# Gepetto/mpc-interface

Measured on AMD Instinct MI355X. Metric: QP assemblies/sec (P,q,G,h), biped N=16 batched, higher is better.
Workload: dtype f64; 1 GPU; C2 biped LIPM N=16 no=36 nc=76, per-instance (A,B)/given/aim, K1 on chip; batch_per_gpu=4096, global_batch=4096, streams=2

## Files before the change

### include/mpcasm.h

```cpp
#ifndef MPCASM_H
#define MPCASM_H

#include <stddef.h>
#include <stdint.h>

#ifdef __cplusplus
extern "C" {
#endif

typedef enum mpcasm_status {
  MPCASM_OK = 0,
  MPCASM_ERR_ARG = -1,
  MPCASM_ERR_PLAN = -2,
  MPCASM_ERR_HIP = -3,
  MPCASM_ERR_NODEVICE = -4,
  MPCASM_ERR_LIMIT = -5
} mpcasm_status;

typedef struct mpcasm_plan mpcasm_plan;


int mpcasm_abi_version(void);
int mpcasm_device_count(void);
int mpcasm_last_hip(void);
const char* mpcasm_status_string(int status);
enum { MPCASM_OPT_PATH = 1, MPCASM_OPT_PHASE_MASK = 2, MPCASM_OPT_RESIDENT_PER_CU = 3, MPCASM_OPT_JIT = 4,
       MPCASM_OPT_P_DIRECT = 5, MPCASM_OPT_RESIDENT_GRID = 6, MPCASM_OPT_JIT_FETCH_RUNS = 7 };
int mpcasm_set_option(int option, int value);
int mpcasm_plan_set_option(mpcasm_plan* plan, int option, int value);
int mpcasm_resident_lds_bytes(const int32_t* h_itab, size_t n_itab, const double* h_dtab, size_t n_dtab,
                              int64_t out[2]);
int mpcasm_jit_check(const int32_t* h_itab, size_t n_itab, const double* h_dtab, size_t n_dtab,
                     char* log, size_t log_capacity);
int mpcasm_fetch_segments(const int32_t* h_itab, size_t n_itab, const double* h_dtab, size_t n_dtab,
                          int limit, int32_t* out, size_t capacity, int64_t* n_words);

int mpcasm_plan_prepare(const mpcasm_plan* plan, int batch);
int mpcasm_jit_stats(int64_t out[3]);

int mpcasm_fill_su(const double* d_A, const double* d_B, double* d_S, double* d_U,
                   int batch, int N, int n, int m, int ltv, void* stream);

// ... 41 lines not shown
                         double* d_out, int batch, void* stream);

int mpcasm_preview_goal_distance(const mpcasm_plan* plan, const double* const* h_src,
                                 const int64_t* h_src_stride, const double* d_given,
                                 const double* d_optim, const double* d_params, const int32_t* d_terms,
                                 int nterms, int ngoals, double* d_out, void* d_work, int batch,
                                 void* stream);

enum { MPCASM_PREVIEW_NONE = 0 , MPCASM_PREVIEW_DIRECT = 1,
       MPCASM_PREVIEW_STAGED = 2 ,
       MPCASM_PREVIEW_BLOCKED = 3  };
int mpcasm_preview_route(const int32_t* h_itab, size_t n_itab, const double* h_dtab, size_t n_dtab,
                         const int64_t* h_src_stride, int nterms, int ngoals, int32_t out[8]);

int mpcasm_sweep_route(const int32_t* h_itab, size_t n_itab, const double* h_dtab, size_t n_dtab, int32_t out[8]);

enum { MPCASM_TILED_SCAN = 1, MPCASM_TILED_TOEPLITZ = 2, MPCASM_TILED_SHARED = 3, MPCASM_TILED_GENERAL = 4 };
enum { MPCASM_TILED_TABLES_NONE = 0, MPCASM_TILED_TABLES_SMALL = 1 ,
       MPCASM_TILED_TABLES_SYSTEM = 2  };
enum { MPCASM_WANT_COST = 1, MPCASM_WANT_CONSTRAINTS = 2 };
int mpcasm_tiled_route(const int32_t* h_itab, size_t n_itab, const double* h_dtab, size_t n_dtab,
                       const int64_t* h_src_stride, int batch, int want, int path, int32_t out[16]);

int mpcasm_gather(const double* d_src, int64_t src_stride, const int32_t* d_index, int nnz,
                  double* d_dst, int batch, void* stream);

enum { MPCASM_BOX_RECENTER = 0, MPCASM_BOX_TRANSLATE, MPCASM_BOX_ROTATE, MPCASM_BOX_SCALE,
       MPCASM_BOX_MARGIN };
int mpcasm_box_transform(double* d_params, int64_t n_params, int batch, const int32_t* d_facets,
                         int nfacets, int op, const double* d_arg, int64_t arg_stride,
// ... 66 lines not shown
```

### mpc-interface_amd/csrc/capi.hip

```cpp
#include <hip/hip_runtime.h>
#include <stdint.h>
#include <stdlib.h>
#include <string.h>

#include <algorithm>
#include <cmath>
#include <mutex>
#include <new>
#include <string>
#include <vector>

#include "jit.h"
#include "kernels.h"

using namespace mpcasm;

namespace mpcasm {
int g_p_direct = 0;
extern int g_path;
extern int g_phase_mask;
extern int g_resident_per_cu, g_resident_grid;
}

struct mpcasm_plan {
// ... 1065 lines not shown
  if (option == MPCASM_OPT_RESIDENT_PER_CU) {
    if (value < 0 || value > 16) return MPCASM_ERR_ARG;
    g_resident_per_cu = value;
    return MPCASM_OK;
  }
  if (option == MPCASM_OPT_JIT_FETCH_RUNS) {
    if (value < 0 || value > FS_MAX) return MPCASM_ERR_ARG;
    g_jit_fetch_runs = value;
    return MPCASM_OK;
  }
  if (option == MPCASM_OPT_RESIDENT_GRID) {
    if (value < 0 || value > (1 << 20)) return MPCASM_ERR_ARG;
    g_resident_grid = value;
    return MPCASM_OK;
  }
  return MPCASM_ERR_ARG;
}

int mpcasm_plan_set_option(mpcasm_plan* plan, int option, int value) {
  if (!plan) return MPCASM_ERR_ARG;
  if (option == MPCASM_OPT_PATH && value >= -1 && value <= 4) plan->opt_path = value;
  else if (option == MPCASM_OPT_JIT && value >= -1 && value <= 2) plan->opt_jit = value;
  else if (option == MPCASM_OPT_RESIDENT_PER_CU && value >= -1 && value <= 16) plan->opt_per_cu = value;
  else if (option == MPCASM_OPT_RESIDENT_GRID && value >= -1 && value <= (1 << 20)) plan->opt_grid = value;
  else return MPCASM_ERR_ARG;
  return MPCASM_OK;
}

const char* mpcasm_status_string(int status) {
  switch (status) {
// ... 349 lines not shown
  PlanDev d;
  memset(&d, 0, sizeof d);
  plan_dev_from_tables(h_itab, &d);
  if (!sweep_eligible(d)) return MPCASM_ERR_ARG;
  SweepChoice c;
  const int choice = sweep_choose(d, h_itab, &c);
  if (choice != MPCASM_OK) return choice;
  out[0] = c.cpt;
  out[1] = c.specialised;
  out[2] = c.pair;
  out[3] = c.per_line;
  out[4] = c.reg_lines;
  out[5] = sweep_lines_ahead(c.cpt);
  out[6] = (int32_t)c.lds;
  out[7] = c.lds > 64 * 1024;
  return MPCASM_OK;
}

int mpcasm_tiled_route(const int32_t* h_itab, size_t n_itab, const double* h_dtab, size_t n_dtab,
                       const int64_t* h_src_stride, int batch, int want, int path, int32_t out[16]) {
  if (!h_itab || (n_dtab && !h_dtab) || !out || batch < 1 || path < -1 || path > 4 || want < 1 || want > 3)
    return MPCASM_ERR_ARG;
  memset(out, 0, 16 * sizeof(int32_t));
  const int rc = validate_plan(h_itab, h_dtab, n_itab, n_dtab);
  if (rc != MPCASM_OK) return rc;
  PlanDev d;
  memset(&d, 0, sizeof d);
  plan_dev_from_tables(h_itab, &d);
  if (d.nsrc && !h_src_stride) return MPCASM_ERR_ARG;
  SrcTable src;
// ... 386 lines not shown
```

### mpc-interface_amd/csrc/kernels.h

```cpp
#pragma once
#include <hip/hip_runtime.h>
#include <stddef.h>
#include <stdint.h>

#include <vector>

#include "../../include/mpcasm.h"
#include "plan_dev.h"
#include "plan_tables.h"

namespace mpcasm {

constexpr int CU_LDS_BYTES = 160 * 1024;
hipError_t allow_whole_lds(const void* fn);

int launch_fill_su(const double* A, const double* B, double* S, double* U, int batch, int N, int n,
                   int m, int ltv, hipStream_t stream, hipError_t* err);

size_t assemble_workspace_bytes(const PlanDev& p, int batch);
int launch_assemble_staged(const PlanDev& p, const SrcTable& src, const double* params,
                           const double* given, double* P, double* q, double* G, double* h,
                           void* work, int batch, hipStream_t stream, hipError_t* err);
bool tiled_eligible(const PlanDev& p);
size_t tiled_workspace_bytes(const PlanDev& p, int batch);
// ... 4 lines not shown
int launch_lti_tables(const PlanDev& p, const SrcTable& src, double* work, int batch,
                      const int32_t* h_itab, SrcTable* eff, hipStream_t stream);
int toeplitz_zero_pad(int N);
struct TiledChoice {
  int form, fused, kp, cb, rows_in_lds, whole_lines, tables, tg, sym;
  int dlen;
  size_t lds;
};
int tiled_choose(const PlanDev& p, const SrcTable& src, const int32_t* h_itab, int path, int batch,
                 bool want_cost, bool want_constraints, bool have_given, bool have_work, TiledChoice* out);
int lti_effective_sources(const PlanDev& p, const SrcTable& src, double* work, const int32_t* h_itab,
                          SrcTable* eff);
bool sweep_eligible(const PlanDev& p);
struct SweepChoice {
  int cpt, specialised, pair, per_line, reg_lines;
  size_t lds;
};
int sweep_choose(const PlanDev& p, const int32_t* h_itab, SweepChoice* out);
int sweep_lines_ahead(int cpt);
int launch_assemble_sweep(const PlanDev& p, const SrcTable& src, const double* params,
                          const double* given, double* P, double* q, double* G, double* h, int batch,
                          hipStream_t stream, hipError_t* err, const int32_t* h_itab);
int launch_preview_direct(const PlanDev& p, const SrcTable& eff, const double* given,
                          const double* optim, double* out, int batch, int num_cus,
                          hipStream_t stream, hipError_t* err, const int32_t* h_itab = nullptr);
int launch_preview_goals(const PlanDev& p, const SrcTable& eff, const double* given, const double* optim,
                         const double* params, long long nparams, const int32_t* terms, int nterms,
                         int ngoals, double* out, int batch, int num_cus, hipStream_t stream,
                         hipError_t* err, const int32_t* h_itab);
int preview_route(const PlanDev& p, const SrcTable& eff, const int32_t* h_itab, int nterms, int ngoals,
                  int32_t out[8]);
int launch_next_given(const PlanDev& p, const SrcTable& eff, const int32_t* map, long long map_words,
// ... 65 lines not shown
```

### mpc-interface_amd/csrc/sweep.hip

```cpp
#include <hip/hip_runtime.h>
#include <stdint.h>

#include <algorithm>

#include "device_common.h"
#include "kernels.h"

namespace mpcasm {

namespace {

constexpr int SW_BLOCK = 256;
constexpr int SW_WAVES = SW_BLOCK / 64;

__device__ __forceinline__ double ldsd(const double* base, int i) { return base[i]; }

struct SweepLds {
  int ab, xbar, gv, lam, par, cvec, lw, ints, total;
  int i_term, i_gptr, i_axis, i_lword, nints;
};
constexpr int LIMW = SW_LIM_WORDS + SW_AXMAX * SW_LAX_WORDS;
constexpr int SW_TERMS_REG = 8;
constexpr int SW_LINES_REG = 8;
constexpr int sweep_lr(int cpt) { return cpt == 1 ? SW_LINES_REG : (cpt == 2 ? 4 : 2); }
__host__ __device__ inline int sweep_abw(int n, int m) { return (n * n + n * m + 1) & ~1; }
__host__ __device__ inline SweepLds sweep_lds(const PlanDev& p, int per_line) {
  const int n = p.sw_n, m = p.sw_m, N = p.sw_horizon, naxes = p.sw_naxes;
  SweepLds x;
  x.ab = 0;
  x.gv = x.ab + N * sweep_abw(n, m);
  x.lw = x.gv + naxes * m * N * SW_NMAX;
  x.xbar = x.lw + (per_line ? p.sw_ngent : p.sw_nlim) * naxes * SW_NMAX;
  x.lam = x.xbar;
  x.par = x.lam + naxes * N * n;
  x.cvec = x.par + p.nparams + 1;
  x.cvec += x.cvec & 1;
  x.ints = x.cvec + p.sw_ncvec * SW_NMAX;
  x.ints += x.ints & 1;
  x.i_term = 0;
  x.i_gptr = x.i_term + p.sw_nterm * SW_TERM_WORDS;
  x.i_axis = x.i_gptr + N + 2;
  x.i_lword = x.i_axis + naxes * SW_AXIS_WORDS;
  x.nints = x.i_lword + p.sw_ngent + SW_LINES_REG;
  x.total = x.ints + (x.nints + 1) / 2;
  x.total += x.total & 1;
  return x;
}

__device__ __forceinline__ double lane_value(double v, int src) { return __shfl(v, src, 64); }

template <int CPT, int NS, int MS, int AS, bool PAIR = false>
__global__ __launch_bounds__(SW_BLOCK) void ltv_sweep_kernel(
    PlanDev p, const double* __restrict__ sysA, long long strideA, const double* __restrict__ sysB,
    long long strideB, const double* __restrict__ params, const double* __restrict__ given,
    double* __restrict__ P, double* __restrict__ q, double* __restrict__ G, double* __restrict__ h,
    int batch, int per_line, int reg_lines) {
  extern __shared__ __attribute__((aligned(16))) double sw[];
  const int tid = threadIdx.x, lane = tid & 63;
  const int wave = __builtin_amdgcn_readfirstlane(tid >> 6);
  const long inst = blockIdx.x;
  if (inst >= batch) return;
  const int n = NS ? NS : p.sw_n, m = MS ? MS : p.sw_m, naxes = AS ? AS : p.sw_naxes;
  const int N = p.sw_horizon, no = p.no, nc = p.nc;
  const int nn = n * n, nm = n * m, abw = sweep_abw(n, m);
  const SweepLds L = sweep_lds(p, per_line);
  double* AB = sw + L.ab;
  double* xbar = sw + L.xbar;
  double* gv = sw + L.gv;
  double* lamT = sw + L.lam;
  double* par = sw + L.par;
  double* cvec = sw + L.cvec;
  double* lw = sw + L.lw;
  int* itb = reinterpret_cast<int*>(sw + L.ints);
// ... 14 lines not shown
    for (int e = tid; e <= p.nparams; e += SW_BLOCK) par[e] = e < p.nparams ? pb[e] : 0.0;
    for (int e = tid; e < p.sw_ncvec * SW_NMAX; e += SW_BLOCK) cvec[e] = (p.dtab + p.sw_doff_cvec)[e];
    auto copy = [&](int dst, int src_off, int count) {
      for (int e = tid; e < count; e += SW_BLOCK) itb[dst + e] = (p.itab + src_off)[e];
    };
    copy(L.i_term, p.off_sw_term, p.sw_nterm * SW_TERM_WORDS);
    copy(L.i_gptr, p.off_sw_gptr, N + 1);
    if (tid == 0) itb[L.i_gptr + N + 1] = nlines;
    copy(L.i_axis, p.off_sw_axis, naxes * SW_AXIS_WORDS);
  }
  int ca[CPT], cj[CPT], cl[CPT];
  double dPc[CPT], dqc[CPT];
  const int32_t* colw = p.itab + p.off_sw_col;
#pragma unroll
  for (int t = 0; t < CPT; ++t) {
    const int c = PAIR ? tid * CPT + t : tid + t * SW_BLOCK;
    ca[t] = -1;
    cj[t] = cl[t] = 0;
    dPc[t] = dqc[t] = 0.0;
    if (c < no) {
      const int w = colw[c];
      ca[t] = w & 255;
      cj[t] = (w >> 8) & 255;
      cl[t] = w >> 16;
      diagonal_of_column(p, pb, c, dPc[t], dqc[t]);
    }
  }
  __syncthreads();

  const int ra = lane >> 4, ri = (lane >> 2) & 3, rj = lane & 3;
  const bool rlive = ra < naxes && ri < n && rj < n;
// ... 158 lines not shown
        if (l + 1 < N) {
          const double* An = AB + (l + 1) * abw;
          double acl[SW_NMAX];
#pragma unroll
          for (int s_ = 0; s_ < SW_NMAX; ++s_) acl[s_] = (xl && s_ < n) ? An[s_ * n + ri] : 0.0;
          acc = fma(acl[0], lane_value(lam, base), acc);
          acc = fma(acl[1], lane_value(lam, base + 4), acc);
          acc = fma(acl[2], lane_value(lam, base + 8), acc);
          acc = fma(acl[3], lane_value(lam, base + 12), acc);
        }
        lam = xl ? acc : 0.0;
        if (xl) lamT[(ra * N + l) * n + ri] = lam;
      }
    }
  }
  if (G != nullptr && wave >= 2) {
    const int wt = tid - 128, WT = SW_BLOCK - 128;
    for (int e = wt; e < nlines + SW_LINES_REG; e += WT) {
      const int2 ge = gent[e < nlines ? e : nlines - 1];
      const int* rec = lims + ge.x * LIMW;
      lword[e] = (rec[SL_OUT0] + ge.y) | (ge.x << 20);
      if (per_line && e < nlines) {
        for (int a = 0; a < naxes; ++a)
          for (int s_ = 0; s_ < SW_NMAX; ++s_) lw[(e * naxes + a) * SW_NMAX + s_] = 0.0;
        for (int ax = 0; ax < rec[SL_NAXES]; ++ax) {
          const int* xr = rec + SW_LIM_WORDS + ax * SW_LAX_WORDS;
          const double ar = par[xr[SX_ARROW] + ge.y * xr[SX_ARROW_STEP]];
          const double* cv = cvec + xr[SX_CVEC];
          for (int s_ = 0; s_ < n; ++s_) lw[(e * naxes + xr[SX_AXIS]) * SW_NMAX + s_] += ar * cv[s_];
        }
      }
// ... 1 lines not shown
    if (!per_line)
      for (int li = wt; li < p.sw_nlim; li += WT) {
        const int* rec = lims + li * LIMW;
        for (int a = 0; a < naxes; ++a)
          for (int s_ = 0; s_ < SW_NMAX; ++s_) lw[(li * naxes + a) * SW_NMAX + s_] = 0.0;
        for (int ax = 0; ax < rec[SL_NAXES]; ++ax) {
          const int* xr = rec + SW_LIM_WORDS + ax * SW_LAX_WORDS;
          const double ar = par[xr[SX_ARROW]];
          const double* cv = cvec + xr[SX_CVEC];
          for (int s_ = 0; s_ < n; ++s_) lw[(li * naxes + xr[SX_AXIS]) * SW_NMAX + s_] += ar * cv[s_];
        }
      }
  }
  __syncthreads();

  if (P != nullptr)
#pragma unroll
    for (int t = 0; t < CPT; ++t) {
      const int c = PAIR ? tid * CPT + t : tid + t * SW_BLOCK;
      if (c < no) {
        const double* Bl = AB + cl[t] * abw + nn;
        const double* lm = lamT + (ca[t] * N + cl[t]) * n;
        double acc = dqc[t];
        for (int s_ = 0; s_ < n; ++s_) acc = fma(Bl[s_ * m + cj[t]], lm[s_], acc);
        q[(size_t)inst * no + c] = acc;
      }
    }

  double* Pb = P + (size_t)inst * no * no;
  double* Gb = G + (size_t)inst * nc * no;
  if (P != nullptr && naxes > 1) {
    const bool wide = (N & 1) == 0 && (no & 1) == 0;
    for (int a = 0; a < naxes; ++a)
      for (int j = 0; j < m; ++j)
        for (int a2 = 0; a2 < naxes; ++a2) {
          if (a2 == a) continue;
          for (int j2 = 0; j2 < m; ++j2) {
            const int col0 = axis[a2 * SW_AXIS_WORDS + 1 + j2];
            double* blk = Pb + (size_t)axis[a * SW_AXIS_WORDS + 1 + j] * no + col0;
            if (wide && (col0 & 1) == 0)
              for (int e = tid * 2; e < N * N; e += SW_BLOCK * 2) {
                const int r = e / N, c = e - r * N;
                *reinterpret_cast<double2*>(blk + (size_t)r * no + c) = double2{0.0, 0.0};
              }
            else
              for (int e = tid; e < N * N; e += SW_BLOCK) {
                const int r = e / N, c = e - r * N;
                blk[(size_t)r * no + c] = 0.0;
              }
          }
        }
  }

  if ((CPT == 1 && tid >= no) || (PAIR && tid * CPT >= no)) return;
  double u[CPT][SW_NMAX];
  double* prow[CPT][SW_MMAX];
  int goff[CPT];
#pragma unroll
  for (int t = 0; t < CPT; ++t) {
    const int c = PAIR ? tid * CPT + t : tid + t * SW_BLOCK;
    const int cat = ca[t] < 0 ? 0 : ca[t];
    goff[t] = cat * m * SW_NMAX;
#pragma unroll
    for (int i = 0; i < SW_NMAX; ++i) u[t][i] = 0.0;
#pragma unroll
    for (int j = 0; j < SW_MMAX; ++j)
      prow[t][j] = Pb + (size_t)(j < m ? axis[cat * SW_AXIS_WORDS + 1 + j] : 0) * no + (c < no ? c : 0);
  }
  constexpr int RLMAX = 4;
  double wreg[RLMAX][CPT][SW_NMAX];
  double* gp[RLMAX];
#pragma unroll
  for (int x = 0; x < RLMAX; ++x) {
    const int word = (G != nullptr && x < reg_lines) ? __builtin_amdgcn_readfirstlane(lword[x]) : 0;
    gp[x] = Gb + (size_t)(word & 0xFFFFF) * no;
#pragma unroll
    for (int t = 0; t < CPT; ++t) {
      const double* wp = lw + (size_t)(word >> 20) * naxes * SW_NMAX + (goff[t] / m);
#pragma unroll
      for (int s_ = 0; s_ < SW_NMAX; ++s_) wreg[x][t][s_] = (x < reg_lines && s_ < n) ? wp[s_] : 0.0;
    }
  }
  constexpr int LR = sweep_lr(CPT);
  int wcur[LR];
#pragma unroll
  for (int x = 0; x < LR; ++x) wcur[x] = G != nullptr ? __builtin_amdgcn_readfirstlane(lword[x]) : 0;
  int e1 = G != nullptr ? __builtin_amdgcn_readfirstlane(gptr[1]) : 0, e0 = 0;
  for (int l = 0; l < N; ++l) {
    const double* Al = AB + l * abw;
    const double* Bl = Al + nn;
    const int e2 = gptr[l + 2];
    double am[SW_NMAX][SW_NMAX];
#pragma unroll
    for (int i = 0; i < SW_NMAX; ++i)
#pragma unroll
      for (int s_ = 0; s_ < SW_NMAX; ++s_) am[i][s_] = (i < n && s_ < n) ? Al[i * n + s_] : 0.0;
#pragma unroll
    for (int t = 0; t < CPT; ++t) {
      double bnow[SW_NMAX], y[SW_NMAX];
#pragma unroll
      for (int i = 0; i < SW_NMAX; ++i) {
        bnow[i] = i < n ? Bl[i * m + cj[t]] : 0.0;
        asm volatile("" : "+v"(bnow[i]));
// ... 13 lines not shown
    }
    if (P != nullptr) {
      double pv[CPT][SW_MMAX];
#pragma unroll
      for (int t = 0; t < CPT; ++t) {
        const double* gl = gv + (size_t)l * naxes * m * SW_NMAX + goff[t];
#pragma unroll
        for (int j = 0; j < SW_MMAX; ++j) {
          double v = (cl[t] == l && cj[t] == j) ? dPc[t] : 0.0;
#pragma unroll
          for (int s_ = 0; s_ < SW_NMAX; ++s_)
            if (s_ < n && j < m) v = fma(gl[j * SW_NMAX + s_], u[t][s_], v);
          pv[t][j] = v;
        }
      }
#pragma unroll
      for (int j = 0; j < SW_MMAX; ++j) {
        if (j >= m) break;
        if constexpr (PAIR) {
          const bool m0 = cl[0] <= l, m1 = cl[1] <= l;
          if (m0 && m1 && prow[1][j] == prow[0][j] + 1) {
            *reinterpret_cast<double2*>(prow[0][j]) = double2{pv[0][j], pv[1][j]};
          } else {
            if (m0) *prow[0][j] = pv[0][j];
            if (m1) *prow[1][j] = pv[1][j];
          }
        } else {
#pragma unroll
          for (int t = 0; t < CPT; ++t) {
            const int c = tid + t * SW_BLOCK;
            if ((CPT == 1 || c < no) && cl[t] <= l) *prow[t][j] = pv[t][j];
          }
        }
#pragma unroll
        for (int t = 0; t < CPT; ++t) prow[t][j] += no;
      }
    }
    if (G != nullptr && reg_lines > 0) {
#pragma unroll
      for (int x = 0; x < RLMAX; ++x) {
        if (x >= reg_lines) break;
        double vv[CPT];
#pragma unroll
        for (int t = 0; t < CPT; ++t) {
          vv[t] = 0.0;
#pragma unroll
          for (int s_ = 0; s_ < SW_NMAX; ++s_)
            if (s_ < n) vv[t] = fma(wreg[x][t][s_], u[t][s_], vv[t]);
        }
        if constexpr (PAIR) {
          store_result(reinterpret_cast<double2*>(gp[x] + tid * 2), double2{vv[0], vv[1]});
        } else {
#pragma unroll
          for (int t = 0; t < CPT; ++t) {
            const int c = tid + t * SW_BLOCK;
            if (CPT == 1 || c < no) store_result(gp[x] + c, vv[t]);
          }
        }
        gp[x] += no;
      }
      for (int e = e0 + reg_lines; e < e1; ++e) {
        const int word = lword[e];
        double* grow = Gb + (size_t)(word & 0xFFFFF) * no;
#pragma unroll
        for (int t = 0; t < CPT; ++t) {
          const int c = PAIR ? tid * CPT + t : tid + t * SW_BLOCK;
          const double* wp = lw + (size_t)(word >> 20) * naxes * SW_NMAX + (goff[t] / m);
          double v = 0.0;
          for (int s_ = 0; s_ < n; ++s_) v = fma(wp[s_], u[t][s_], v);
          if (CPT == 1 || c < no) store_result(grow + c, v);
        }
      }
    } else if (G != nullptr) {
      const int cnt = e1 - e0;
      const int first_next = e1;
      double wv[LR][CPT][SW_NMAX];
#pragma unroll
      for (int x = 0; x < LR; ++x) {
        const int word = wcur[x];
        const int slot = per_line ? e0 + (x < cnt ? x : 0) : (word >> 20);
#pragma unroll
        for (int t = 0; t < CPT; ++t) {
          const double* wp = lw + (size_t)slot * naxes * SW_NMAX + (goff[t] / m);
#pragma unroll
          for (int s_ = 0; s_ < SW_NMAX; ++s_) wv[x][t][s_] = s_ < n ? wp[s_] : 0.0;
        }
      }
      int wnext[LR];
#pragma unroll
      for (int x = 0; x < LR; ++x) wnext[x] = lword[first_next + x];
#pragma unroll
      for (int x = 0; x < LR; ++x) {
        if (x >= cnt) break;
        double* grow = Gb + (size_t)(wcur[x] & 0xFFFFF) * no;
#pragma unroll
        for (int t = 0; t < CPT; ++t) {
          const int c = PAIR ? tid * CPT + t : tid + t * SW_BLOCK;
          double v = 0.0;
#pragma unroll
          for (int s_ = 0; s_ < SW_NMAX; ++s_)
            if (s_ < n) v = fma(wv[x][t][s_], u[t][s_], v);
          if (CPT == 1 || c < no) store_result(grow + c, v);
        }
      }
      for (int e = e0 + LR; e < e1; ++e) {
        const int word = lword[e];
        const int slot = per_line ? e : (word >> 20);
        double* grow = Gb + (size_t)(word & 0xFFFFF) * no;
#pragma unroll
        for (int t = 0; t < CPT; ++t) {
          const int c = PAIR ? tid * CPT + t : tid + t * SW_BLOCK;
          const double* wp = lw + (size_t)slot * naxes * SW_NMAX + (goff[t] / m);
          double v = 0.0;
          for (int s_ = 0; s_ < n; ++s_) v = fma(wp[s_], u[t][s_], v);
          if (CPT == 1 || c < no) store_result(grow + c, v);
        }
      }
#pragma unroll
      for (int x = 0; x < LR; ++x) wcur[x] = __builtin_amdgcn_readfirstlane(wnext[x]);
    }
    e0 = e1;
    e1 = __builtin_amdgcn_readfirstlane(e2);
  }
  if (P == nullptr) return;

  double z[CPT][SW_NMAX];
#pragma unroll
  for (int t = 0; t < CPT; ++t)
#pragma unroll
    for (int i = 0; i < SW_NMAX; ++i) z[t][i] = 0.0;
  for (int l = N - 1; l >= 0; --l) {
    const double* An = AB + (l + 1 < N ? l + 1 : l) * abw;
    const double* Bl = AB + l * abw + nn;
    double at[SW_NMAX][SW_NMAX], bm[SW_NMAX][SW_MMAX], bv[CPT][SW_MMAX];
#pragma unroll
    for (int i = 0; i < SW_NMAX; ++i)
#pragma unroll
      for (int s_ = 0; s_ < SW_NMAX; ++s_) at[s_][i] = (i < n && s_ < n) ? An[s_ * n + i] : 0.0;
#pragma unroll
    for (int s_ = 0; s_ < SW_NMAX; ++s_)
#pragma unroll
      for (int j = 0; j < SW_MMAX; ++j) bm[s_][j] = (s_ < n && j < m) ? Bl[s_ * m + j] : 0.0;
#pragma unroll
    for (int t = 0; t < CPT; ++t) {
      const int c = PAIR ? tid * CPT + t : tid + t * SW_BLOCK;
      const double* gl = gv + (size_t)l * naxes * m * SW_NMAX + goff[t] + cj[t] * SW_NMAX;
      double gnow[SW_NMAX], y[SW_NMAX];
#pragma unroll
      for (int i = 0; i < SW_NMAX; ++i) {
        gnow[i] = i < n ? gl[i] : 0.0;
        asm volatile("" : "+v"(gnow[i]));
      }
#pragma unroll
      for (int i = 0; i < SW_NMAX; ++i) {
        y[i] = 0.0;
        if (i < n) {
#pragma unroll
          for (int s_ = 0; s_ < SW_NMAX; ++s_)
            if (s_ < n) y[i] = fma(at[s_][i], z[t][s_], y[i]);
          y[i] = cl[t] == l ? gnow[i] : y[i];
// ... 19 lines not shown
      for (int j = 0; j < SW_MMAX; ++j) {
        if (j >= m) break;
        const bool m0 = cl[0] > l, m1 = cl[1] > l;
        if (m0 && m1 && prow[1][j] == prow[0][j] + 1) {
          *reinterpret_cast<double2*>(prow[0][j]) = double2{bv[0][j], bv[1][j]};
        } else {
          if (m0) *prow[0][j] = bv[0][j];
          if (m1) *prow[1][j] = bv[1][j];
        }
      }
    }
  }
}

}

bool sweep_eligible(const PlanDev& p) { return p.sw_ok != 0; }
int sweep_lines_ahead(int cpt) { return sweep_lr(cpt); }

int sweep_choose(const PlanDev& p, const int32_t* h_itab, SweepChoice* out) {
  *out = SweepChoice{};
  const int n = p.sw_n, m = p.sw_m, naxes = p.sw_naxes;
  if (n < 1 || n > SW_NMAX || m < 1 || m > SW_MMAX || naxes < 1 || naxes > SW_AXMAX ||
      naxes * n * n > 64 || p.no > SW_BLOCK * 4)
    return MPCASM_ERR_LIMIT;
  int per_line = p.sw_nlim >= (1 << 11) || p.nc >= (1 << 20);
  if (h_itab == nullptr) return MPCASM_ERR_ARG;
  for (int li = 0; li < p.sw_nlim && !per_line; ++li) {
    const int32_t* rec = h_itab + p.off_sw_lim + li * LIMW;
    for (int ax = 0; ax < rec[SL_NAXES]; ++ax) per_line |= rec[SW_LIM_WORDS + ax * SW_LAX_WORDS + SX_ARROW_STEP] != 0;
// ... 19 lines not shown
      }
    }
    reg_lines = R;
  }
  const size_t lds = (size_t)sweep_lds(p, per_line).total * sizeof(double);
  if (lds > (size_t)RESIDENT_LDS_LIMIT) return MPCASM_ERR_LIMIT;
  const bool even = (p.no & 1) == 0 && (p.sw_horizon & 1) == 0;
  const bool lipm = n == 3 && m == 1 && naxes == 2;
  SweepChoice c;
  c.per_line = per_line;
  c.reg_lines = reg_lines;
  c.lds = lds;
  c.pair = even && p.no <= SW_BLOCK * 2;
  c.cpt = c.pair ? 2 : (p.no <= SW_BLOCK ? 1 : (p.no <= SW_BLOCK * 2 ? 2 : 4));
  c.specialised = lipm && (c.pair || c.cpt == 1);
  *out = c;
  return MPCASM_OK;
}

int launch_assemble_sweep(const PlanDev& p, const SrcTable& src, const double* params,
                          const double* given, double* P, double* q, double* G, double* h, int batch,
                          hipStream_t stream, hipError_t* err, const int32_t* h_itab) {
  SweepChoice c;
  const int rc = sweep_choose(p, h_itab, &c);
  if (rc != MPCASM_OK) return rc;
  const int per_line = c.per_line, reg_lines = c.reg_lines;
  const size_t lds = c.lds;
  const double* A = src.ptr[p.sw_src_a];
  const double* Bm = src.ptr[p.sw_src_b];
  const long long sa = src.stride[p.sw_src_a], sb = src.stride[p.sw_src_b];
#define MPCASM_SWEEP_CASE(CPT, NS, MS, AS, PAIR)                                                       \
  if (c.cpt == CPT && c.specialised == (NS != 0) && c.pair == (int)PAIR) {                             \
    auto kernel = ltv_sweep_kernel<CPT, NS, MS, AS, PAIR>;                                             \
    if (lds > 64 * 1024) {                                                                             \
      *err = allow_whole_lds(reinterpret_cast<const void*>(kernel));                                   \
      if (*err != hipSuccess) return MPCASM_ERR_HIP;                                                   \
    }                                                                                                  \
    hipLaunchKernelGGL(kernel, dim3((unsigned)batch), dim3(SW_BLOCK), lds, stream, p, A, sa, Bm, sb,   \
                       params, given, P, q, G, h, batch, per_line, reg_lines);                         \
    *err = hipGetLastError();                                                                          \
    return *err == hipSuccess ? MPCASM_OK : MPCASM_ERR_HIP;                                            \
  }
  MPCASM_SWEEP_CASE(2, 3, 1, 2, true)
  MPCASM_SWEEP_CASE(1, 3, 1, 2, false)
  MPCASM_SWEEP_CASE(2, 0, 0, 0, true)
  MPCASM_SWEEP_CASE(1, 0, 0, 0, false)
  MPCASM_SWEEP_CASE(2, 0, 0, 0, false)
  MPCASM_SWEEP_CASE(4, 0, 0, 0, false)
#undef MPCASM_SWEEP_CASE
  return MPCASM_ERR_LIMIT;
}

}
```

### mpc-interface_amd/mpcasm/capi.py

```python
import ctypes
import os

_HERE = os.path.dirname(os.path.abspath(__file__))
LIB_PATH = os.environ.get("MPCASM_LIB") or os.path.join(_HERE, "libmpcasm.so")

OK = 0
ERR_LIMIT = -5
OPT_PATH = 1
OPT_PHASE_MASK = 2
OPT_RESIDENT_PER_CU = 3
OPT_RESIDENT_GRID = 6
OPT_P_DIRECT = 5
OPT_JIT_FETCH_RUNS = 7
OPT_JIT = 4
PHASE_DEFAULT = 0xBF
PHASE_STAMPS = 0x40
STATUS = {
    0: "MPCASM_OK",
    -1: "MPCASM_ERR_ARG",
    -2: "MPCASM_ERR_PLAN",
    -3: "MPCASM_ERR_HIP",
    -4: "MPCASM_ERR_NODEVICE",
    -5: "MPCASM_ERR_LIMIT",
}
QP_SOLVED, QP_MAX_ITER, QP_PRIMAL_INFEASIBLE, QP_DUAL_INFEASIBLE, QP_NON_CVX = 1, -2, -3, -4, -7
QP_STATUS = {
    1: "MPCASM_QP_SOLVED",
    -2: "MPCASM_QP_MAX_ITER",
# ... 22 lines not shown
                                      _void_p]),
    "mpcasm_plan_create": (ctypes.c_int, [_void_p, ctypes.c_size_t, _void_p, ctypes.c_size_t,
                                          ctypes.POINTER(_void_p)]),
    "mpcasm_plan_destroy": (ctypes.c_int, [_void_p]),
    "mpcasm_resident_lds_bytes": (ctypes.c_int, [_void_p, ctypes.c_size_t, _void_p, ctypes.c_size_t,
                                                 ctypes.POINTER(ctypes.c_int64)]),
    "mpcasm_jit_check": (ctypes.c_int, [_void_p, ctypes.c_size_t, _void_p, ctypes.c_size_t,
                                        ctypes.c_char_p, ctypes.c_size_t]),
    "mpcasm_fetch_segments": (ctypes.c_int, [_void_p, ctypes.c_size_t, _void_p, ctypes.c_size_t, ctypes.c_int,
                                             _void_p, ctypes.c_size_t, ctypes.POINTER(ctypes.c_int64)]),
    "mpcasm_preview_route": (ctypes.c_int, [_void_p, ctypes.c_size_t, _void_p, ctypes.c_size_t,
                                            ctypes.POINTER(ctypes.c_int64), ctypes.c_int, ctypes.c_int,
                                            ctypes.POINTER(ctypes.c_int32)]),
    "mpcasm_sweep_route": (ctypes.c_int, [_void_p, ctypes.c_size_t, _void_p, ctypes.c_size_t,
                                          ctypes.POINTER(ctypes.c_int32)]),
    "mpcasm_tiled_route": (ctypes.c_int, [_void_p, ctypes.c_size_t, _void_p, ctypes.c_size_t,
                                          ctypes.POINTER(ctypes.c_int64), ctypes.c_int, ctypes.c_int, ctypes.c_int,
                                          ctypes.POINTER(ctypes.c_int32)]),
    "mpcasm_plan_sizes": (ctypes.c_int, [_void_p, ctypes.POINTER(ctypes.c_int64)]),
    "mpcasm_plan_csc_sizes": (ctypes.c_int, [_void_p, ctypes.POINTER(ctypes.c_int64)]),
    "mpcasm_plan_set_option": (ctypes.c_int, [_void_p, ctypes.c_int, ctypes.c_int]),
    "mpcasm_assemble_indexed": (ctypes.c_int, [_void_p, ctypes.POINTER(_void_p),
                                               ctypes.POINTER(ctypes.c_int64), _void_p, _void_p, _void_p,
                                               _void_p, _void_p, _void_p, _void_p, _void_p, ctypes.c_int,
                                               _void_p]),
    "mpcasm_plan_last_kernel": (ctypes.c_int, [_void_p]),
    "mpcasm_plan_prepare": (ctypes.c_int, [_void_p, ctypes.c_int]),
    "mpcasm_jit_stats": (ctypes.c_int, [ctypes.POINTER(ctypes.c_int64)]),
    "mpcasm_workspace_bytes": (ctypes.c_int, [_void_p, ctypes.c_int,
                                              ctypes.POINTER(ctypes.c_size_t)]),
# ... 107 lines not shown
```

### mpc-interface_amd/mpcasm/engine.py

```python
import collections
import ctypes

import numpy as np

from . import capi
from .plan import compile_plan, is_causal, rollout_rows, rollout_sizes


def _torch():
    import torch

    return torch


def require_device():
    torch = _torch()
    if not torch.cuda.is_available():
        raise RuntimeError(
            "mpcasm: no HIP device is visible; the QP-assembly path runs only on the GPU "
            "(there is no CPU fallback)")
    capi.load()
    return torch


# ... 236 lines not shown
        int(nterms), int(ngoals), out)
    if rc == capi.ERR_LIMIT:
        return None
    capi.check(rc, "mpcasm_preview_route")
    return tuple(int(x) for x in out)


def sweep_route(plan):
    out = (ctypes.c_int32 * 8)()
    itab, dtab = np.ascontiguousarray(plan.itab), np.ascontiguousarray(plan.dtab)
    capi.check(capi.load().mpcasm_sweep_route(
        itab.ctypes.data, itab.size, dtab.ctypes.data if dtab.size else None, dtab.size, out), "mpcasm_sweep_route")
    return tuple(int(x) for x in out)


TiledRoute = collections.namedtuple(
    "TiledRoute", "form fused kp cb rows_in_lds whole_lines lds whole_lds tables tg sym")


def tiled_route(plan, batch, src_stride=None, want=capi.WANT_COST | capi.WANT_CONSTRAINTS, path=0):
    out = (ctypes.c_int32 * 16)()
    itab, dtab = np.ascontiguousarray(plan.itab), np.ascontiguousarray(plan.dtab)
    n = len(plan.sources)
    strides = (ctypes.c_int64 * max(n, 1))(*([0] * n if src_stride is None else [int(x) for x in src_stride]))
    capi.check(capi.load().mpcasm_tiled_route(
        itab.ctypes.data, itab.size, dtab.ctypes.data if dtab.size else None, dtab.size, strides, int(batch),
        int(want), int(path), out), "mpcasm_tiled_route")
    return TiledRoute(*(int(x) for x in out[:11]))


# ... 400 lines not shown
                x.data_ptr() if x is not None else None, out.data_ptr(), work.data_ptr(), n,
                _stream_handle(torch, stream))
        capi.check(rc, "mpcasm_preview_direct")
        return out

    def preview_route(self, goals=False):
        nterms = ngoals = 0
        if goals is not False and goals is not None:
            table, names = self.goal_terms(goals)
            nterms, ngoals = int(table.shape[0]), len(names)
        return preview_route(self.plan, self._src_stride, nterms, ngoals)

    def sweep_route(self):
        return sweep_route(self.plan)

    def tiled_route(self, want_cost=True, want_constraints=True, count=None):
        want = (capi.WANT_COST if want_cost else 0) | (capi.WANT_CONSTRAINTS if want_constraints and self.nc else 0)
        return tiled_route(self.plan, self.batch if count is None else int(count), self._src_stride, want,
                           getattr(self, "_opt_path", -1))

    def given_map(self, rules):
        torch = self._torch
        rows, values = given_map_records(self.plan, rules)
        lib, words = capi.load(), ctypes.c_int64()
        args = (self._handle, rows.ctypes.data, values.ctypes.data, self.ng)
        capi.check(lib.mpcasm_given_map_compile(*args, None, 0, ctypes.byref(words)), "mpcasm_given_map_compile")
        host = np.zeros(max(words.value, 1), dtype=np.int32)
        capi.check(lib.mpcasm_given_map_compile(*args, host.ctypes.data, host.size, ctypes.byref(words)),
                   "mpcasm_given_map_compile")
        return GivenMap(torch.as_tensor(host, device=self.device), int(words.value), rows, values, self.plan)
# ... 185 lines not shown
```

Before: 177.8 million assemblies/s.

## Assemble P rows directly in sweep kernel via LDS parking and split forward/backward halves

Adds a ROWS mode to the LTV sweep kernel that writes P as full rows instead of columns. Half-horizon partial results are parked in LDS so the forward and backward sweeps can fill the symmetric halves, and the separate symmetrisation pass is skipped. A SPLIT variant runs the backward recursion in the second half of the block at the same time as the forward sweep in the first half. It is on by default when the parked data fits an 80 KB LDS budget. The cost is extra LDS (which may reduce occupancy) and many more kernel instantiations.

```diff
diff --git a/include/mpcasm.h b/include/mpcasm.h
--- a/include/mpcasm.h
+++ b/include/mpcasm.h
@@ -25,7 +25,8 @@
 int mpcasm_last_hip(void);
 const char* mpcasm_status_string(int status);
 enum { MPCASM_OPT_PATH = 1, MPCASM_OPT_PHASE_MASK = 2, MPCASM_OPT_RESIDENT_PER_CU = 3, MPCASM_OPT_JIT = 4,
-       MPCASM_OPT_P_DIRECT = 5, MPCASM_OPT_RESIDENT_GRID = 6, MPCASM_OPT_JIT_FETCH_RUNS = 7 };
+       MPCASM_OPT_P_DIRECT = 5, MPCASM_OPT_RESIDENT_GRID = 6, MPCASM_OPT_JIT_FETCH_RUNS = 7,
+       MPCASM_OPT_SWEEP_ROWS = 8 };
 int mpcasm_set_option(int option, int value);
 int mpcasm_plan_set_option(mpcasm_plan* plan, int option, int value);
 int mpcasm_resident_lds_bytes(const int32_t* h_itab, size_t n_itab, const double* h_dtab, size_t n_dtab,
@@ -97,6 +98,8 @@
                          const int64_t* h_src_stride, int nterms, int ngoals, int32_t out[8]);
 
 int mpcasm_sweep_route(const int32_t* h_itab, size_t n_itab, const double* h_dtab, size_t n_dtab, int32_t out[8]);
+int mpcasm_sweep_rows_route(const int32_t* h_itab, size_t n_itab, const double* h_dtab, size_t n_dtab,
+                            int32_t out[4]);
 
 enum { MPCASM_TILED_SCAN = 1, MPCASM_TILED_TOEPLITZ = 2, MPCASM_TILED_SHARED = 3, MPCASM_TILED_GENERAL = 4 };
 enum { MPCASM_TILED_TABLES_NONE = 0, MPCASM_TILED_TABLES_SMALL = 1 ,
diff --git a/mpc-interface_amd/csrc/capi.hip b/mpc-interface_amd/csrc/capi.hip
--- a/mpc-interface_amd/csrc/capi.hip
+++ b/mpc-interface_amd/csrc/capi.hip
@@ -1103,6 +1103,11 @@
     g_resident_grid = value;
     return MPCASM_OK;
   }
+  if (option == MPCASM_OPT_SWEEP_ROWS) {
+    if (value < 0 || value > 2) return MPCASM_ERR_ARG;
+    g_sweep_rows = value;
+    return MPCASM_OK;
+  }
   return MPCASM_ERR_ARG;
 }
 
@@ -1482,6 +1487,26 @@
   out[5] = sweep_lines_ahead(c.cpt);
   out[6] = (int32_t)c.lds;
   out[7] = c.lds > 64 * 1024;
+  return MPCASM_OK;
+}
+
+int mpcasm_sweep_rows_route(const int32_t* h_itab, size_t n_itab, const double* h_dtab, size_t n_dtab,
+                            int32_t out[4]) {
+  if (!h_itab || (n_dtab && !h_dtab) || !out) return MPCASM_ERR_ARG;
+  memset(out, 0, 4 * sizeof(int32_t));
+  const int rc = validate_plan(h_itab, h_dtab, n_itab, n_dtab);
+  if (rc != MPCASM_OK) return rc;
+  PlanDev d;
+  memset(&d, 0, sizeof d);
+  plan_dev_from_tables(h_itab, &d);
+  if (!sweep_eligible(d)) return MPCASM_ERR_ARG;
+  SweepChoice c;
+  const int choice = sweep_choose(d, h_itab, &c);
+  if (choice != MPCASM_OK) return choice;
+  out[0] = c.rows;
+  out[1] = c.rows_h;
+  out[2] = (int32_t)c.park;
+  out[3] = (int32_t)c.lds;
   return MPCASM_OK;
 }
 
diff --git a/mpc-interface_amd/csrc/kernels.h b/mpc-interface_amd/csrc/kernels.h
--- a/mpc-interface_amd/csrc/kernels.h
+++ b/mpc-interface_amd/csrc/kernels.h
@@ -42,8 +42,10 @@
 bool sweep_eligible(const PlanDev& p);
 struct SweepChoice {
   int cpt, specialised, pair, per_line, reg_lines;
-  size_t lds;
+  int rows, rows_h, split;
+  size_t lds, lds_pieces, park;
 };
+extern int g_sweep_rows;
 int sweep_choose(const PlanDev& p, const int32_t* h_itab, SweepChoice* out);
 int sweep_lines_ahead(int cpt);
 int launch_assemble_sweep(const PlanDev& p, const SrcTable& src, const double* params,
diff --git a/mpc-interface_amd/csrc/sweep.hip b/mpc-interface_amd/csrc/sweep.hip
--- a/mpc-interface_amd/csrc/sweep.hip
+++ b/mpc-interface_amd/csrc/sweep.hip
@@ -20,6 +20,7 @@
   int i_term, i_gptr, i_axis, i_lword, nints;
 };
 constexpr int LIMW = SW_LIM_WORDS + SW_AXMAX * SW_LAX_WORDS;
+constexpr size_t SWEEP_ROWS_LDS = 80 * 1024;
 constexpr int SW_TERMS_REG = 8;
 constexpr int SW_LINES_REG = 8;
 constexpr int sweep_lr(int cpt) { return cpt == 1 ? SW_LINES_REG : (cpt == 2 ? 4 : 2); }
@@ -47,9 +48,11 @@
   return x;
 }
 
+__host__ __device__ inline int sweep_park_stride(int H, bool pair) { return pair ? (H + 1) & ~1 : H; }
+
 __device__ __forceinline__ double lane_value(double v, int src) { return __shfl(v, src, 64); }
 
-template <int CPT, int NS, int MS, int AS, bool PAIR = false>
+template <int CPT, int NS, int MS, int AS, bool PAIR = false, bool ROWS = false, bool SPLIT = false>
 __global__ __launch_bounds__(SW_BLOCK) void ltv_sweep_kernel(
     PlanDev p, const double* __restrict__ sysA, long long strideA, const double* __restrict__ sysB,
     long long strideB, const double* __restrict__ params, const double* __restrict__ given,
@@ -57,6 +60,8 @@
     int batch, int per_line, int reg_lines) {
   extern __shared__ __attribute__((aligned(16))) double sw[];
   const int tid = threadIdx.x, lane = tid & 63;
+  const int ctid = SPLIT ? (tid & (SW_BLOCK / 2 - 1)) : tid;
+  const bool bwd = SPLIT && tid >= SW_BLOCK / 2;
   const int wave = __builtin_amdgcn_readfirstlane(tid >> 6);
   const long inst = blockIdx.x;
   if (inst >= batch) return;
@@ -101,7 +106,7 @@
   const int32_t* colw = p.itab + p.off_sw_col;
 #pragma unroll
   for (int t = 0; t < CPT; ++t) {
-    const int c = PAIR ? tid * CPT + t : tid + t * SW_BLOCK;
+    const int c = PAIR ? ctid * CPT + t : ctid + t * SW_BLOCK;
     ca[t] = -1;
     cj[t] = cl[t] = 0;
     dPc[t] = dqc[t] = 0.0;
@@ -290,7 +295,7 @@
       }
     }
   }
-  if (G != nullptr && wave >= 2) {
+  if (G != nullptr && wave >= 2 && nlines > 0) {
     const int wt = tid - 128, WT = SW_BLOCK - 128;
     for (int e = wt; e < nlines + SW_LINES_REG; e += WT) {
       const int2 ge = gent[e < nlines ? e : nlines - 1];
@@ -322,10 +327,10 @@
   }
   __syncthreads();
 
-  if (P != nullptr)
+  if (P != nullptr && !bwd)
 #pragma unroll
     for (int t = 0; t < CPT; ++t) {
-      const int c = PAIR ? tid * CPT + t : tid + t * SW_BLOCK;
+      const int c = PAIR ? ctid * CPT + t : ctid + t * SW_BLOCK;
       if (c < no) {
         const double* Bl = AB + cl[t] * abw + nn;
         const double* lm = lamT + (ca[t] * N + cl[t]) * n;
@@ -337,7 +342,7 @@
 
   double* Pb = P + (size_t)inst * no * no;
   double* Gb = G + (size_t)inst * nc * no;
-  if (P != nullptr && naxes > 1) {
+  if (!ROWS && P != nullptr && naxes > 1) {
     const bool wide = (N & 1) == 0 && (no & 1) == 0;
     for (int a = 0; a < naxes; ++a)
       for (int j = 0; j < m; ++j)
@@ -360,13 +365,14 @@
         }
   }
 
-  if ((CPT == 1 && tid >= no) || (PAIR && tid * CPT >= no)) return;
+  const bool dead = (CPT == 1 && ctid >= no) || (PAIR && ctid * CPT >= no);
+  if (!SPLIT && dead) return;
   double u[CPT][SW_NMAX];
   double* prow[CPT][SW_MMAX];
   int goff[CPT];
 #pragma unroll
   for (int t = 0; t < CPT; ++t) {
-    const int c = PAIR ? tid * CPT + t : tid + t * SW_BLOCK;
+    const int c = PAIR ? ctid * CPT + t : ctid + t * SW_BLOCK;
     const int cat = ca[t] < 0 ? 0 : ca[t];
     goff[t] = cat * m * SW_NMAX;
 #pragma unroll
@@ -375,6 +381,105 @@
     for (int j = 0; j < SW_MMAX; ++j)
       prow[t][j] = Pb + (size_t)(j < m ? axis[cat * SW_AXIS_WORDS + 1 + j] : 0) * no + (c < no ? c : 0);
   }
+  const int H = (N + 1) >> 1, Hp = sweep_park_stride(H, PAIR);
+  const int psq = H * Hp;
+  double* park = sw + L.total;
+  int plo[CPT], phi[CPT];
+  int rowcol[SW_AXMAX * SW_MMAX];
+  double z[CPT][SW_NMAX];
+#pragma unroll
+  for (int t = 0; t < CPT; ++t)
+#pragma unroll
+    for (int i = 0; i < SW_NMAX; ++i) z[t][i] = 0.0;
+  if constexpr (ROWS) {
+#pragma unroll
+    for (int t = 0; t < CPT; ++t) {
+      const int cat = ca[t] < 0 ? 0 : ca[t];
+      const int base = (cat * m * m + cj[t]) * psq;
+      const int lo = cl[t], hi = cl[t] >= H ? cl[t] - H : 0;
+      plo[t] = base + (PAIR ? (lo >> 1) + (lo & 1) * (Hp >> 1) : lo);
+      phi[t] = base + (PAIR ? (hi >> 1) + (hi & 1) * (Hp >> 1) : hi);
+    }
+#pragma unroll
+    for (int a = 0; a < SW_AXMAX; ++a)
+#pragma unroll
+      for (int j = 0; j < SW_MMAX; ++j)
+        rowcol[a * SW_MMAX + j] =
+            (a < naxes && j < m) ? __builtin_amdgcn_readfirstlane(axis[a * SW_AXIS_WORDS + 1 + j]) : 0;
+  }
+  auto write_rows = [&](int l, const double (&val)[CPT][SW_MMAX]) {
+#pragma unroll
+    for (int a = 0; a < SW_AXMAX; ++a) {
+      if (a >= naxes) break;
+#pragma unroll
+      for (int j = 0; j < SW_MMAX; ++j) {
+        if (j >= m) break;
+        double* row = Pb + (size_t)(rowcol[a * SW_MMAX + j] + l) * no;
+        if constexpr (PAIR) {
+          store_result(reinterpret_cast<double2*>(row + ctid * 2),
+                       double2{ca[0] == a ? val[0][j] : 0.0, ca[1] == a ? val[1][j] : 0.0});
+        } else {
+#pragma unroll
+          for (int t = 0; t < CPT; ++t) {
+            const int c = ctid + t * SW_BLOCK;
+            if (CPT == 1 || c < no) store_result(row + c, ca[t] == a ? val[t][j] : 0.0);
+          }
+        }
+      }
+    }
+  };
+  auto backward_step = [&](int lb) {
+    const double* An = AB + (lb + 1 < N ? lb + 1 : lb) * abw;
+    const double* Bb = AB + lb * abw + nn;
+    double at[SW_NMAX][SW_NMAX], bm[SW_NMAX][SW_MMAX], bv[CPT][SW_MMAX];
+#pragma unroll
+    for (int i = 0; i < SW_NMAX; ++i)
+#pragma unroll
+      for (int s_ = 0; s_ < SW_NMAX; ++s_) at[s_][i] = (i < n && s_ < n) ? An[s_ * n + i] : 0.0;
+#pragma unroll
+    for (int s_ = 0; s_ < SW_NMAX; ++s_)
+#pragma unroll
+      for (int j = 0; j < SW_MMAX; ++j) bm[s_][j] = (s_ < n && j < m) ? Bb[s_ * m + j] : 0.0;
+#pragma unroll
+    for (int t = 0; t < CPT; ++t) {
+      const int c = PAIR ? ctid * CPT + t : ctid + t * SW_BLOCK;
+      const double* gl = gv + (size_t)lb * naxes * m * SW_NMAX + goff[t] + cj[t] * SW_NMAX;
+      double gnow[SW_NMAX], y[SW_NMAX];
+#pragma unroll
+      for (int i = 0; i < SW_NMAX; ++i) {
+        gnow[i] = i < n ? gl[i] : 0.0;
+        asm volatile("" : "+v"(gnow[i]));
+      }
+#pragma unroll
+      for (int i = 0; i < SW_NMAX; ++i) {
+        y[i] = 0.0;
+        if (i < n) {
+#pragma unroll
+          for (int s_ = 0; s_ < SW_NMAX; ++s_)
+            if (s_ < n) y[i] = fma(at[s_][i], z[t][s_], y[i]);
+          y[i] = cl[t] == lb ? gnow[i] : y[i];
+        }
+      }
+#pragma unroll
+      for (int i = 0; i < SW_NMAX; ++i) z[t][i] = y[i];
+#pragma unroll
+      for (int j = 0; j < SW_MMAX; ++j) {
+        double v = 0.0;
+#pragma unroll
+        for (int s_ = 0; s_ < SW_NMAX; ++s_)
+          if (s_ < n && j < m) v = fma(bm[s_][j], z[t][s_], v);
+        bv[t][j] = v;
+        if (j < m && (CPT == 1 || c < no)) {
+          if (lb >= H) {
+            if (cl[t] > lb) park[phi[t] + j * m * psq + (lb - H) * Hp] = v;
+          } else if (cl[t] <= lb) {
+            bv[t][j] = park[plo[t] + j * m * psq + lb * Hp];
+          }
+        }
+      }
+    }
+    if (lb < H) write_rows(lb, bv);
+  };
   constexpr int RLMAX = 4;
   double wreg[RLMAX][CPT][SW_NMAX];
   double* gp[RLMAX];
@@ -394,7 +499,9 @@
 #pragma unroll
   for (int x = 0; x < LR; ++x) wcur[x] = G != nullptr ? __builtin_amdgcn_readfirstlane(lword[x]) : 0;
   int e1 = G != nullptr ? __builtin_amdgcn_readfirstlane(gptr[1]) : 0, e0 = 0;
-  for (int l = 0; l < N; ++l) {
+  for (int ph = 0; ph < (SPLIT ? 2 : 1); ++ph) {
+  if (!bwd && !(SPLIT && dead))
+  for (int l = SPLIT && ph ? H : 0; l < (SPLIT && !ph ? H : N); ++l) {
     const double* Al = AB + l * abw;
     const double* Bl = Al + nn;
     const int e2 = gptr[l + 2];
@@ -438,9 +545,29 @@
           pv[t][j] = v;
         }
       }
+      if constexpr (ROWS) {
+        if (l < H) {
+#pragma unroll
+          for (int t = 0; t < CPT; ++t) {
+            const int c = PAIR ? ctid * CPT + t : ctid + t * SW_BLOCK;
+#pragma unroll
+            for (int j = 0; j < SW_MMAX; ++j)
+              if (j < m && (CPT == 1 || c < no) && cl[t] <= l) park[plo[t] + j * m * psq + l * Hp] = pv[t][j];
+          }
+        } else {
+#pragma unroll
+          for (int t = 0; t < CPT; ++t) {
+            const int c = PAIR ? ctid * CPT + t : ctid + t * SW_BLOCK;
+#pragma unroll
+            for (int j = 0; j < SW_MMAX; ++j)
+              if (j < m && (CPT == 1 || c < no) && cl[t] > l) pv[t][j] = park[phi[t] + j * m * psq + (l - H) * Hp];
+          }
+          write_rows(l, pv);
+        }
+      }
 #pragma unroll
       for (int j = 0; j < SW_MMAX; ++j) {
-        if (j >= m) break;
+        if (ROWS || j >= m) break;
         if constexpr (PAIR) {
           const bool m0 = cl[0] <= l, m1 = cl[1] <= l;
           if (m0 && m1 && prow[1][j] == prow[0][j] + 1) {
@@ -452,7 +579,7 @@
         } else {
 #pragma unroll
           for (int t = 0; t < CPT; ++t) {
-            const int c = tid + t * SW_BLOCK;
+            const int c = ctid + t * SW_BLOCK;
             if ((CPT == 1 || c < no) && cl[t] <= l) *prow[t][j] = pv[t][j];
           }
         }
@@ -473,11 +600,11 @@
             if (s_ < n) vv[t] = fma(wreg[x][t][s_], u[t][s_], vv[t]);
         }
         if constexpr (PAIR) {
-          store_result(reinterpret_cast<double2*>(gp[x] + tid * 2), double2{vv[0], vv[1]});
+          store_result(reinterpret_cast<double2*>(gp[x] + ctid * 2), double2{vv[0], vv[1]});
         } else {
 #pragma unroll
           for (int t = 0; t < CPT; ++t) {
-            const int c = tid + t * SW_BLOCK;
+            const int c = ctid + t * SW_BLOCK;
             if (CPT == 1 || c < no) store_result(gp[x] + c, vv[t]);
           }
         }
@@ -488,7 +615,7 @@
         double* grow = Gb + (size_t)(word & 0xFFFFF) * no;
 #pragma unroll
         for (int t = 0; t < CPT; ++t) {
-          const int c = PAIR ? tid * CPT + t : tid + t * SW_BLOCK;
+          const int c = PAIR ? ctid * CPT + t : ctid + t * SW_BLOCK;
           const double* wp = lw + (size_t)(word >> 20) * naxes * SW_NMAX + (goff[t] / m);
           double v = 0.0;
           for (int s_ = 0; s_ < n; ++s_) v = fma(wp[s_], u[t][s_], v);
@@ -519,7 +646,7 @@
         double* grow = Gb + (size_t)(wcur[x] & 0xFFFFF) * no;
 #pragma unroll
         for (int t = 0; t < CPT; ++t) {
-          const int c = PAIR ? tid * CPT + t : tid + t * SW_BLOCK;
+          const int c = PAIR ? ctid * CPT + t : ctid + t * SW_BLOCK;
           double v = 0.0;
 #pragma unroll
           for (int s_ = 0; s_ < SW_NMAX; ++s_)
@@ -533,7 +660,7 @@
         double* grow = Gb + (size_t)(word & 0xFFFFF) * no;
 #pragma unroll
         for (int t = 0; t < CPT; ++t) {
-          const int c = PAIR ? tid * CPT + t : tid + t * SW_BLOCK;
+          const int c = PAIR ? ctid * CPT + t : ctid + t * SW_BLOCK;
           const double* wp = lw + (size_t)slot * naxes * SW_NMAX + (goff[t] / m);
           double v = 0.0;
           for (int s_ = 0; s_ < n; ++s_) v = fma(wp[s_], u[t][s_], v);
@@ -545,14 +672,17 @@
     }
     e0 = e1;
     e1 = __builtin_amdgcn_readfirstlane(e2);
-  }
-  if (P == nullptr) return;
-
-  double z[CPT][SW_NMAX];
-#pragma unroll
-  for (int t = 0; t < CPT; ++t)
-#pragma unroll
-    for (int i = 0; i < SW_NMAX; ++i) z[t][i] = 0.0;
+    if constexpr (ROWS && !SPLIT)
+      if (P != nullptr) backward_step(N - 1 - l);
+  }
+    if constexpr (SPLIT) {
+      if (bwd && !dead && P != nullptr)
+        for (int lb = (ph ? H : N) - 1; lb >= (ph ? 0 : H); --lb) backward_step(lb);
+      if (ph == 0) __syncthreads();
+    }
+  }
+  if (ROWS || P == nullptr) return;
+
   for (int l = N - 1; l >= 0; --l) {
     const double* An = AB + (l + 1 < N ? l + 1 : l) * abw;
     const double* Bl = AB + l * abw + nn;
@@ -567,7 +697,7 @@
       for (int j = 0; j < SW_MMAX; ++j) bm[s_][j] = (s_ < n && j < m) ? Bl[s_ * m + j] : 0.0;
 #pragma unroll
     for (int t = 0; t < CPT; ++t) {
-      const int c = PAIR ? tid * CPT + t : tid + t * SW_BLOCK;
+      const int c = PAIR ? ctid * CPT + t : ctid + t * SW_BLOCK;
       const double* gl = gv + (size_t)l * naxes * m * SW_NMAX + goff[t] + cj[t] * SW_NMAX;
       double gnow[SW_NMAX], y[SW_NMAX];
 #pragma unroll
@@ -617,6 +747,8 @@
 }
 
 }
+
+int g_sweep_rows = 0;
 
 bool sweep_eligible(const PlanDev& p) { return p.sw_ok != 0; }
 int sweep_lines_ahead(int cpt) { return sweep_lr(cpt); }
@@ -666,6 +798,17 @@
   c.pair = even && p.no <= SW_BLOCK * 2;
   c.cpt = c.pair ? 2 : (p.no <= SW_BLOCK ? 1 : (p.no <= SW_BLOCK * 2 ? 2 : 4));
   c.specialised = lipm && (c.pair || c.cpt == 1);
+  c.rows_h = (p.sw_horizon + 1) / 2;
+  c.park = sizeof(double) * (size_t)naxes * m * m * c.rows_h * sweep_park_stride(c.rows_h, c.pair != 0);
+  c.lds_pieces = lds;
+  const size_t with_rows = lds + c.park;
+  const bool can_split = (c.pair && c.specialised && p.no <= SW_BLOCK) || (c.cpt == 1 && p.no <= SW_BLOCK / 2);
+  if (g_sweep_rows == 2)
+    c.rows = c.cpt != 4 && with_rows <= (size_t)RESIDENT_LDS_LIMIT;
+  else
+    c.rows = g_sweep_rows == 0 && can_split && with_rows <= SWEEP_ROWS_LDS;
+  c.split = c.rows && can_split;
+  if (c.rows) c.lds = with_rows;
   *out = c;
   return MPCASM_OK;
 }
@@ -676,14 +819,17 @@
   SweepChoice c;
   const int rc = sweep_choose(p, h_itab, &c);
   if (rc != MPCASM_OK) return rc;
+  if (p.nc == 0) G = h = nullptr;
   const int per_line = c.per_line, reg_lines = c.reg_lines;
-  const size_t lds = c.lds;
+  const bool rows = c.rows && P != nullptr;
+  const size_t lds = rows ? c.lds : c.lds_pieces;
   const double* A = src.ptr[p.sw_src_a];
   const double* Bm = src.ptr[p.sw_src_b];
   const long long sa = src.stride[p.sw_src_a], sb = src.stride[p.sw_src_b];
-#define MPCASM_SWEEP_CASE(CPT, NS, MS, AS, PAIR)                                                       \
-  if (c.cpt == CPT && c.specialised == (NS != 0) && c.pair == (int)PAIR) {                             \
-    auto kernel = ltv_sweep_kernel<CPT, NS, MS, AS, PAIR>;                                             \
+#define MPCASM_SWEEP_CASE(CPT, NS, MS, AS, PAIR, ROWS, SPLIT)                                          \
+  if (c.cpt == CPT && c.specialised == (NS != 0) && c.pair == (int)PAIR && rows == ROWS &&             \
+      (rows && c.split) == SPLIT) {                                                                    \
+    auto kernel = ltv_sweep_kernel<CPT, NS, MS, AS, PAIR, ROWS, SPLIT>;                                \
     if (lds > 64 * 1024) {                                                                             \
       *err = allow_whole_lds(reinterpret_cast<const void*>(kernel));                                   \
       if (*err != hipSuccess) return MPCASM_ERR_HIP;                                                   \
@@ -693,12 +839,20 @@
     *err = hipGetLastError();                                                                          \
     return *err == hipSuccess ? MPCASM_OK : MPCASM_ERR_HIP;                                            \
   }
-  MPCASM_SWEEP_CASE(2, 3, 1, 2, true)
-  MPCASM_SWEEP_CASE(1, 3, 1, 2, false)
-  MPCASM_SWEEP_CASE(2, 0, 0, 0, true)
-  MPCASM_SWEEP_CASE(1, 0, 0, 0, false)
-  MPCASM_SWEEP_CASE(2, 0, 0, 0, false)
-  MPCASM_SWEEP_CASE(4, 0, 0, 0, false)
+  MPCASM_SWEEP_CASE(2, 3, 1, 2, true, true, true)
+  MPCASM_SWEEP_CASE(1, 3, 1, 2, false, true, true)
+  MPCASM_SWEEP_CASE(1, 0, 0, 0, false, true, true)
+  MPCASM_SWEEP_CASE(2, 3, 1, 2, true, true, false)
+  MPCASM_SWEEP_CASE(1, 3, 1, 2, false, true, false)
+  MPCASM_SWEEP_CASE(2, 0, 0, 0, true, true, false)
+  MPCASM_SWEEP_CASE(1, 0, 0, 0, false, true, false)
+  MPCASM_SWEEP_CASE(2, 0, 0, 0, false, true, false)
+  MPCASM_SWEEP_CASE(2, 3, 1, 2, true, false, false)
+  MPCASM_SWEEP_CASE(1, 3, 1, 2, false, false, false)
+  MPCASM_SWEEP_CASE(2, 0, 0, 0, true, false, false)
+  MPCASM_SWEEP_CASE(1, 0, 0, 0, false, false, false)
+  MPCASM_SWEEP_CASE(2, 0, 0, 0, false, false, false)
+  MPCASM_SWEEP_CASE(4, 0, 0, 0, false, false, false)
 #undef MPCASM_SWEEP_CASE
   return MPCASM_ERR_LIMIT;
 }
diff --git a/mpc-interface_amd/mpcasm/capi.py b/mpc-interface_amd/mpcasm/capi.py
--- a/mpc-interface_amd/mpcasm/capi.py
+++ b/mpc-interface_amd/mpcasm/capi.py
@@ -12,6 +12,7 @@
 OPT_RESIDENT_GRID = 6
 OPT_P_DIRECT = 5
 OPT_JIT_FETCH_RUNS = 7
+OPT_SWEEP_ROWS = 8
 OPT_JIT = 4
 PHASE_DEFAULT = 0xBF
 PHASE_STAMPS = 0x40
@@ -64,6 +65,8 @@
                                             ctypes.POINTER(ctypes.c_int32)]),
     "mpcasm_sweep_route": (ctypes.c_int, [_void_p, ctypes.c_size_t, _void_p, ctypes.c_size_t,
                                           ctypes.POINTER(ctypes.c_int32)]),
+    "mpcasm_sweep_rows_route": (ctypes.c_int, [_void_p, ctypes.c_size_t, _void_p, ctypes.c_size_t,
+                                               ctypes.POINTER(ctypes.c_int32)]),
     "mpcasm_tiled_route": (ctypes.c_int, [_void_p, ctypes.c_size_t, _void_p, ctypes.c_size_t,
                                           ctypes.POINTER(ctypes.c_int64), ctypes.c_int, ctypes.c_int, ctypes.c_int,
                                           ctypes.POINTER(ctypes.c_int32)]),
diff --git a/mpc-interface_amd/mpcasm/engine.py b/mpc-interface_amd/mpcasm/engine.py
--- a/mpc-interface_amd/mpcasm/engine.py
+++ b/mpc-interface_amd/mpcasm/engine.py
@@ -274,6 +274,15 @@
     return tuple(int(x) for x in out)
 
 
+def sweep_rows_route(plan):
+    out = (ctypes.c_int32 * 4)()
+    itab, dtab = np.ascontiguousarray(plan.itab), np.ascontiguousarray(plan.dtab)
+    capi.check(capi.load().mpcasm_sweep_rows_route(
+        itab.ctypes.data, itab.size, dtab.ctypes.data if dtab.size else None, dtab.size, out),
+        "mpcasm_sweep_rows_route")
+    return tuple(int(x) for x in out)
+
+
 TiledRoute = collections.namedtuple(
     "TiledRoute", "form fused kp cb rows_in_lds whole_lines lds whole_lds tables tg sym")
 
@@ -704,6 +713,9 @@
     def sweep_route(self):
         return sweep_route(self.plan)
 
+    def sweep_rows_route(self):
+        return sweep_rows_route(self.plan)
+
     def tiled_route(self, want_cost=True, want_constraints=True, count=None):
         want = (capi.WANT_COST if want_cost else 0) | (capi.WANT_CONSTRAINTS if want_constraints and self.nc else 0)
         return tiled_route(self.plan, self.batch if count is None else int(count), self._src_stride, want,
```

Result: no change. 178.1 million assemblies/s, median of 2 (+0.2%).
